# zjykzj/YOLOv4

Measured on AMD Instinct MI355X. Metric: images/sec fwd+bwd @608x608 bs=64 per GPU (YOLOv4 training step: forward + YOLOLoss + backward), higher is better.
Workload: dtype f32

## Files before the change

### yolov4_amd/csrc/conv_planes.hip

```cpp
#include <stdlib.h>
#include <type_traits>
#include "common.h"
#include "conv_geom.h"

namespace {

typedef _Float16 f16x8 __attribute__((ext_vector_type(8)));
typedef float f32x4v __attribute__((ext_vector_type(4)));

__device__ __host__ __forceinline__ unsigned pl_scale_exp(unsigned amax_bits) {
    const unsigned e = (amax_bits >> 23) & 0xffu;
    if (e == 0u || e == 255u) return 127u;
    int se = 268 - (int)e;
    if (se < 2) se = 2;
    if (se > 252) se = 252;
    return (unsigned)se;
}
__device__ __forceinline__ float pl_scale(const unsigned* amax) { return __uint_as_float(pl_scale_exp(amax ? *amax : 0u) << 23); }
__device__ __forceinline__ float pl_unscale(const unsigned* amax) { return __uint_as_float((254u - pl_scale_exp(amax ? *amax : 0u)) << 23); }

struct PlaneConvGeom {
    const unsigned char* src;
    const unsigned char* wt;
    float* dst; long long ldd;
// ... 226 lines not shown
            step(std::integral_constant<int, 0>{}, kt);
            step(std::integral_constant<int, 1>{}, kt + 1);
        }
        if (kt < KT) step(std::integral_constant<int, 0>{}, kt);
    }

    const float un = BF ? 1.0f : pl_unscale(g.src_amax) * pl_unscale(g.wt_amax);
    const float un1 = un * (1.0f / 2048.0f);
    auto result = [&](int i, int j, int e) -> float {
        if constexpr (BF) return acc0[i][j][e];
        else return acc0[i][j][e] * un + acc1[i][j][e] * un1;
    };
    {
        const unsigned drow = (unsigned)g.ldd * 4u, rrow = (unsigned)g.ldr * 4u;
        const long long row0 = (long long)mt * BM;
        const unsigned long long left = (unsigned long long)(g.M - row0);
        const unsigned long long dby = left * drow, rby = g.ldr ? left * rrow : (unsigned long long)g.N * 4ull;
        const __amdgpu_buffer_rsrc_t drs = y4_make_rsrc(reinterpret_cast<char*>(g.dst) + row0 * (long long)drow, (unsigned)(dby < 0xfffffff0ull ? dby : 0xfffffff0ull));
        const __amdgpu_buffer_rsrc_t rrs = y4_make_rsrc(g.res ? reinterpret_cast<const char*>(g.res) + row0 * (long long)rrow : nullptr,
                                                        g.res ? (unsigned)(rby < 0xfffffff0ull ? rby : 0xfffffff0ull) : 0u);
        int lane_e = lane;
        asm volatile("" : "+v"(lane_e));
        const int fr = lane_e & 15, kq = lane_e >> 4;
        const int colb = n0 + wn * WTN + fr;
        const bool allc = n0 + BN <= g.N;
        if constexpr (DG2) {
            const __amdgpu_buffer_rsrc_t xrs = y4_make_rsrc(g.dst, (unsigned)((unsigned long long)g.B * g.Hfull * g.Wfull * drow));
#pragma unroll
            for (int i = 0; i < TM; ++i) {
                const int m0 = mt * BM + wm * WTM + 16 * i + 4 * kq;
                int b = m0 / pix_per_img;
                const int rem = m0 - b * pix_per_img;
                int hc = rem / g.Wd, wc = rem - hc * g.Wd;
#pragma unroll
                for (int e = 0; e < 4; ++e) {
                    const bool rok = m0 + e < g.M;
                    const unsigned po = (unsigned)((b * g.Hfull + 2 * hc + g.cls_ph) * g.Wfull + 2 * wc + g.cls_pw) * drow + (unsigned)colb * 4u;
#pragma unroll
                    for (int j = 0; j < TN; ++j) {
                        const float v = result(i, j, e);
                        const bool cok = rok && (allc || colb + 16 * j < g.N);
                        __builtin_amdgcn_raw_buffer_store_b32(__builtin_bit_cast(unsigned, v), xrs, (int)(cok ? po + 64u * j : 0xffffffffu), 0, PL_ST_POL);
                    }
                    if (++wc == g.Wd) { wc = 0; if (++hc == g.Hd) { hc = 0; ++b; } }
                }
            }
        } else if constexpr (!YB) {
        if (g.res) {
            constexpr int EB = TM > 4 ? 1 : 4;
#pragma unroll
            for (int i = 0; i < TM; ++i) {
                const unsigned rl = (unsigned)(wm * WTM + 16 * i + 4 * kq);
                const unsigned dvo = rl * drow + (unsigned)colb * 4u, rvo = rl * rrow + (unsigned)colb * 4u;
#pragma unroll
                for (int e0 = 0; e0 < 4; e0 += EB) {
                    float rv[EB][TN];
#pragma unroll
                    for (int e = 0; e < EB; ++e)
#pragma unroll
                        for (int j = 0; j < TN; ++j) {
                            const bool cok = allc || colb + 16 * j < g.N;
                            rv[e][j] = __builtin_bit_cast(float, __builtin_amdgcn_raw_buffer_load_b32(rrs, (int)(cok ? rvo + 64u * j : 0xffffffffu), (int)((e0 + e) * rrow), 0));
                        }
#pragma unroll
                    for (int e = 0; e < EB; ++e)
#pragma unroll
                        for (int j = 0; j < TN; ++j) {
                            const float v = result(i, j, e0 + e);
                            acc0[i][j][e0 + e] = v;
                            const bool cok = allc || colb + 16 * j < g.N;
                            __builtin_amdgcn_raw_buffer_store_b32(__builtin_bit_cast(unsigned, v + rv[e][j]), drs, (int)(cok ? dvo + 64u * j : 0xffffffffu), (int)((e0 + e) * drow), PL_ST_POL);
                        }
                }
            }
        } else {
#pragma unroll
            for (int i = 0; i < TM; ++i) {
                const unsigned rl = (unsigned)(wm * WTM + 16 * i + 4 * kq);
                const unsigned dvo = rl * drow + (unsigned)colb * 4u;
#pragma unroll
                for (int e = 0; e < 4; ++e)
#pragma unroll
                    for (int j = 0; j < TN; ++j) {
                        const float v = result(i, j, e);
                        acc0[i][j][e] = v;
                        const bool cok = allc || colb + 16 * j < g.N;
                        __builtin_amdgcn_raw_buffer_store_b32(__builtin_bit_cast(unsigned, v), drs, (int)(cok ? dvo + 64u * j : 0xffffffffu), (int)(e * drow), PL_ST_POL);
                    }
            }
        }
        } else {
            float csum[TN], cssum[TN];
#pragma unroll
            for (int j = 0; j < TN; ++j) { csum[j] = 0.f; cssum[j] = 0.f; }
#pragma unroll
            for (int i = 0; i < TM; ++i) {
                const unsigned rl = (unsigned)(wm * WTM + 16 * i + 4 * kq);
                const unsigned dvo = rl * drow + (unsigned)colb * 2u;
#pragma unroll
                for (int e = 0; e < 4; ++e)
#pragma unroll
                    for (int j = 0; j < TN; ++j) {
                        const float v = result(i, j, e);
                        unsigned u = __builtin_bit_cast(unsigned, v);
                        u = (u + 0x7fffu + ((u >> 16) & 1u)) & 0xffff0000u;
                        const float vr = __builtin_bit_cast(float, u);
                        csum[j] += vr; cssum[j] += vr * vr;
                        const unsigned nb = (unsigned)__builtin_amdgcn_update_dpp(0, (int)u, 0xB1, 0xf, 0xf, true);
                        const bool cok = (allc || colb + 16 * j < g.N) && !(fr & 1);
                        __builtin_amdgcn_raw_buffer_store_b32((u >> 16) | nb, drs, (int)(cok ? dvo + 32u * j : 0xffffffffu), (int)(e * drow), PL_ST_POL);
                    }
                __builtin_amdgcn_sched_barrier(0);
            }
#pragma unroll
            for (int j = 0; j < TN; ++j) { acc0[0][j][0] = csum[j]; acc0[0][j][1] = cssum[j]; }
        }
    }
    if (g.stats) {
        __syncthreads();
        float* red = reinterpret_cast<float*>(smem);
#pragma unroll
        for (int j = 0; j < TN; ++j) {
            float cs = 0.f, css = 0.f;
            if constexpr (YB) {
                cs = acc0[0][j][0]; css = acc0[0][j][1];
            } else {
#pragma unroll
                for (int i = 0; i < TM; ++i)
#pragma unroll
                    for (int e = 0; e < 4; ++e) { const float v = acc0[i][j][e]; cs += v; css += v * v; }
            }
            cs += __shfl_xor(cs, 16, 64); css += __shfl_xor(css, 16, 64);
            cs += __shfl_xor(cs, 32, 64); css += __shfl_xor(css, 32, 64);
            if (kq == 0) {
                const int c = wn * WTN + j * 16 + fr;
                red[(wm * BN + c) * 2 + 0] = cs;
                red[(wm * BN + c) * 2 + 1] = css;
            }
        }
        __syncthreads();
        for (int c = tid; c < BN; c += NTHR) {
            float cs = 0.f, css = 0.f;
#pragma unroll
            for (int w = 0; w < WM; ++w) { cs += red[(w * BN + c) * 2]; css += red[(w * BN + c) * 2 + 1]; }
            const int n = n0 + c;
            if (n < g.N) {
                g.stats[((long long)mt * 2 + 0) * g.N + n] = cs;
                g.stats[((long long)mt * 2 + 1) * g.N + n] = css;
            }
        }
    }
}

struct PlaneWgradGeom {
    const unsigned char* x;
    const unsigned char* dy;
    float* out;
    int B, H, W, Cin, Cout, k, pad, M, J;
    int ldy_ch;
    int ntn, ntj, splits, steps_per_split;
    unsigned long long x_total_bytes, dy_total_bytes;
    const unsigned* x_amax; const unsigned* dy_amax;
};

typedef __fp16 trh4 __attribute__((__vector_size__(4 * sizeof(__fp16))));
__device__ __forceinline__ f16x8 tr_frag(const unsigned char* p) {
    typedef __attribute__((address_space(3))) trh4* lp;
    const trh4 a = __builtin_amdgcn_ds_read_tr16_b64_v4f16((lp)(p));
    const trh4 b = __builtin_amdgcn_ds_read_tr16_b64_v4f16((lp)(p + 4 * PROW));
    f16x8 r;
#pragma unroll
    for (int e = 0; e < 4; ++e) { r[e] = (_Float16)a[e]; r[4 + e] = (_Float16)b[e]; }
    return r;
}

template <int N> __device__ __forceinline__ void pl_wait_vm() {
    static_assert(N == 0 || N == 3 || N == 4 || N == 6 || N == 8 || N == 12, "add the literal");
    if constexpr (N == 0) asm volatile("s_waitcnt vmcnt(0)" ::: "memory");
    else if constexpr (N == 3) asm volatile("s_waitcnt vmcnt(3)" ::: "memory");
    else if constexpr (N == 4) asm volatile("s_waitcnt vmcnt(4)" ::: "memory");
    else if constexpr (N == 6) asm volatile("s_waitcnt vmcnt(6)" ::: "memory");
    else if constexpr (N == 8) asm volatile("s_waitcnt vmcnt(8)" ::: "memory");
    else asm volatile("s_waitcnt vmcnt(12)" ::: "memory");
}

template <int TN_, int TJ_, bool BF, int SD = 1>
__global__ __launch_bounds__(512, 1) void wgrad_planes_mfma(const PlaneWgradGeom g) {
    constexpr int NWAVE = 8, WN2 = 2, WJ = 4;
    constexpr int BAR = 2;
    constexpr int CH = BF ? 64 : 32, CSH = BF ? 6 : 5;
    constexpr int WTN = TN_ / WN2, WTJ = TJ_ / WJ, TM = WTN / 16, TN = WTJ / 16;
    static_assert(TN == 4 && (TM == 4 || (BF && TM == 8)), "wave tile 64 x 64 (bf16 also 128 x 64)");
    constexpr int A_BYTES = (TN_ / CH) * 32 * PROW, B_BYTES = (TJ_ / CH) * 32 * PROW, STAGE = A_BYTES + B_BYTES, NSTAGE = 3;
    constexpr int PA = A_BYTES / 1024 / NWAVE, PB = B_BYTES / 1024 / NWAVE, NDMA = PA + PB;
    static_assert(PA >= 1 && PB >= 1 && (NDMA == 6 || NDMA == 3 || NDMA == 4), "DMA pieces per wave and K-step (counted vmcnt literals)");
    typedef float accv __attribute__((ext_vector_type(4)));
    extern __shared__ __attribute__((aligned(1024))) unsigned char smem[];

    const int tid = threadIdx.x, lane = tid & 63;
    const int wave = __builtin_amdgcn_readfirstlane(tid >> 6);
    const int wn2 = wave >> 2, wj = wave & 3;
    const int tiles = g.ntn * g.ntj;
    int bid = y4_xcd_remap(blockIdx.x, tiles * g.splits);
    const int split = bid / tiles;
    bid -= split * tiles;
    const int tn = bid / g.ntj, tj = bid - tn * g.ntj;
    const int n0 = tn * TN_, j0 = tj * TJ_;
    const int CC = g.Cin >> CSH;

    const int steps_total = (g.M + 31) >> 5;
    const int s0 = split * g.steps_per_split;
    int KT = steps_total - s0;
    if (KT > g.steps_per_split) KT = g.steps_per_split;
    if (KT < 0) KT = 0;
    const long long P0 = (long long)s0 * 32;

    const unsigned pitch_x = (unsigned)g.Cin * 4u, pitch_dy = (unsigned)g.ldy_ch * 4u;
    const long long back = SD == 1 ? (long long)g.pad * g.W + g.pad : 2ll * g.W + 2ll * g.W + 1;
    const long long Pw = SD * SD * P0 > back ? SD * SD * P0 - back : 0;
    const unsigned long long dy_skip = (unsigned long long)P0 * pitch_dy, x_skip = (unsigned long long)Pw * pitch_x;
    const unsigned long long dy_left = g.dy_total_bytes > dy_skip ? g.dy_total_bytes - dy_skip : 0ull;
    const unsigned long long x_left = g.x_total_bytes > x_skip ? g.x_total_bytes - x_skip : 0ull;
    const __amdgpu_buffer_rsrc_t dy_rsrc = y4_make_rsrc(g.dy + dy_skip, (unsigned)(dy_left < 0xfffffff0ull ? dy_left : 0xfffffff0ull));
    const __amdgpu_buffer_rsrc_t x_rsrc = y4_make_rsrc(g.x + x_skip, (unsigned)(x_left < 0xfffffff0ull ? x_left : 0xfffffff0ull));
    const unsigned OOB = 0xffffffffu;

    const int lr = lane >> 3, pos = lane & 7;
    unsigned a_voff[PA];
#pragma unroll
    for (int i = 0; i < PA; ++i) {
        const int a = wave * PA + i;
        const int chunk = a >> 2, p = (a & 3) * 8 + lr;
        const int gsw = ((p >> 1) & 1) | (((p >> 3) & 1) << 1);
        const unsigned srcoff = (unsigned)((((pos >> 1) ^ gsw) << 5) + ((pos & 1) << 4));
        a_voff[i] = (n0 + chunk * CH) < g.Cout ? (unsigned)p * pitch_dy + (unsigned)(n0 / CH + chunk) * 128u + srcoff : OOB;
    }
    const int xp = (wave & 3) * 8 + lr;
    unsigned x_const[PB];
    unsigned x_pk = 0u;
    {
        const int gsw = ((xp >> 1) & 1) | (((xp >> 3) & 1) << 1);
        const unsigned srcoff = (unsigned)((((pos >> 1) ^ gsw) << 5) + ((pos & 1) << 4));
#pragma unroll
        for (int i = 0; i < PB; ++i) {
            const int jg = j0 / CH + (wave >> 2) * PB + i;
            const bool ok = jg * CH < g.J;
            const int tap = ok ? jg / CC : 0;
            const int c32 = jg - tap * CC;
            const int r = tap / g.k, q = tap - r * g.k;
            x_pk |= (unsigned)((ok ? r - g.pad + 2 : 15) | ((q - g.pad + 2) << 4)) << (8 * i);
            x_const[i] = (unsigned)((long long)(SD * SD * P0 - Pw) * pitch_x) + (unsigned)(((r - g.pad) * (SD * g.W) + (q - g.pad)) * (int)pitch_x) +
                         (unsigned)c32 * 128u + srcoff;
        }
    }
    int lp = (int)P0 + xp;
    int lh, lw;
    {
        const long long hw = (long long)g.H * g.W;
        const long long rem = (long long)lp % hw;
        lh = (int)(rem / g.W); lw = (int)(rem - (long long)lh * g.W);
    }
    unsigned lbase = (unsigned)xp * pitch_x;
    unsigned ldy = 0u;
    typedef __attribute__((address_space(3))) void* lds_ptr;
    auto issue = [&](int stage, auto P0c, auto P1c) {
        constexpr int p0 = decltype(P0c)::value, p1 = decltype(P1c)::value;
        unsigned char* st = smem + stage * STAGE;
#pragma unroll
        for (int p = p0; p < p1; ++p) {
            if (p < PA) {
                const unsigned vo = a_voff[p] == OOB ? OOB : a_voff[p] + ldy;
                __builtin_amdgcn_raw_ptr_buffer_load_lds(dy_rsrc, (lds_ptr)(st + (wave * PA + p) * 1024), 16, (int)vo, 0, 0, 0);
            } else {
                const int i = p - PA;
                const int dh = (int)((x_pk >> (8 * i)) & 15u) - 2, dw = (int)((x_pk >> (8 * i + 4)) & 15u) - 2;
                const bool ok = lp < g.M && (unsigned)(SD * lh + dh) < (unsigned)(SD * g.H) && (unsigned)(SD * lw + dw) < (unsigned)(SD * g.W);
                const unsigned lb = SD == 1 ? lbase : (unsigned)(4 * (lp - (int)P0) - 2 * lw) * pitch_x;
                const unsigned vo = ok ? lb + x_const[i] : OOB;
                const int b = ((wave >> 2) * PB + i) * 4 + (wave & 3);
                __builtin_amdgcn_raw_ptr_buffer_load_lds(x_rsrc, (lds_ptr)(st + A_BYTES + b * 1024), 16, (int)vo, 0, 0, 0);
            }
        }
        if constexpr (p1 == NDMA) {
            lp += 32; lbase += 32u * pitch_x; ldy += 32u * pitch_dy;
            lw += 32;
            while (lw >= g.W) { lw -= g.W; if (++lh == g.H) lh = 0; }
        }
    };
    using I0 = std::integral_constant<int, 0>;
    using I6 = std::integral_constant<int, NDMA>;

    accv acc0[TM][TN], acc1[BF ? 1 : TM][BF ? 1 : TN];
#pragma unroll
    for (int i = 0; i < TM; ++i)
#pragma unroll
        for (int j = 0; j < TN; ++j)
#pragma unroll
            for (int e = 0; e < 4; ++e) {
                acc0[i][j][e] = 0.f;
                if constexpr (!BF) acc1[i][j][e] = 0.f;
            }

    const int grp = lane >> 4, qrow = (lane >> 2) & 3, pp = lane & 3;
    const int gsw = ((qrow >> 1) & 1) | ((grp & 1) << 1);
    const int rowoff = (8 * grp + qrow) * PROW + pp * 8;
    int segoff[4];
// ... 222 lines not shown
        const unsigned lrow = (unsigned)(wave * 32 + 4 * fh);
#pragma unroll
        for (int j = 0; j < NT; ++j) {
            const int n = j * 32 + fr;
            const bool nok = n < g.N;
            if constexpr (YB) {
                const bool st = nok && !(fr & 1);
#pragma unroll
                for (int q = 0; q < 4; ++q) {
                    const unsigned vo = st ? (lrow + 8u * q) * drow + (unsigned)n * 2u : 0xffffffffu;
#pragma unroll
                    for (int r = 0; r < 4; ++r) {
                        const unsigned me = (unsigned)pl_bf16_bits(acc[j][q * 4 + r]);
                        const float vr = __uint_as_float(me << 16);
                        cs[j] += vr; css[j] += vr * vr;
                        const unsigned nb = pair_swap_u(me);
                        __builtin_amdgcn_raw_buffer_store_b32(me | (nb << 16), drs, (int)vo, (int)(r * drow), PL_ST_POL);
                    }
                }
            } else {
#pragma unroll
                for (int q = 0; q < 4; ++q) {
                    const unsigned vo = nok ? (lrow + 8u * q) * drow + (unsigned)n * 4u : 0xffffffffu;
                    const unsigned ro = nok ? (lrow + 8u * q) * rrow + (unsigned)n * 4u : 0xffffffffu;
                    float rr[4] = {0.f, 0.f, 0.f, 0.f};
                    if (g.res) {
#pragma unroll
                        for (int r = 0; r < 4; ++r)
                            rr[r] = __builtin_bit_cast(float, __builtin_amdgcn_raw_buffer_load_b32(rrs, (int)ro, (int)(r * rrow), 0));
                    }
#pragma unroll
                    for (int r = 0; r < 4; ++r) {
                        const float v = acc[j][q * 4 + r];
                        cs[j] += v; css[j] += v * v;
                        __builtin_amdgcn_raw_buffer_store_b32(__builtin_bit_cast(unsigned, v + rr[r]), drs, (int)vo, (int)(r * drow), PL_ST_POL);
                    }
                }
            }
        }
    };
    int tile = blockIdx.x;
    if (tile < mtiles) load(ra0, tile);
    while (tile < mtiles) {
        const int t1 = tile + gridDim.x;
        if (t1 < mtiles) load(ra1, t1);
        mma(ra0); epilogue(tile);
        if (t1 >= mtiles) break;
        const int t2 = t1 + gridDim.x;
        if (t2 < mtiles) load(ra0, t2);
        mma(ra1); epilogue(t1);
        tile = t2;
    }
    if (g.stats) {
        __syncthreads();
        float* red = reinterpret_cast<float*>(smem_sb);
#pragma unroll
        for (int j = 0; j < NT; ++j) {
            float a = cs[j], b = css[j];
            a += __shfl_xor(a, 32, 64);
            b += __shfl_xor(b, 32, 64);
            if (fh == 0) { red[(wave * N32 + j * 32 + fr) * 2] = a; red[(wave * N32 + j * 32 + fr) * 2 + 1] = b; }
        }
        __syncthreads();
        for (int c = tid; c < N32; c += NTHR) {
            float a = 0.f, b = 0.f;
#pragma unroll
            for (int w = 0; w < NW; ++w) { a += red[(w * N32 + c) * 2]; b += red[(w * N32 + c) * 2 + 1]; }
            if (c < g.N) {
                g.stats[((long long)blockIdx.x * 2 + 0) * g.N + c] = a;
                g.stats[((long long)blockIdx.x * 2 + 1) * g.N + c] = b;
            }
        }
    }
}

template <int KS, int NT, int NW, bool YB>
static int launch_stream_bf16(const PlaneConvGeom& g0, hipStream_t st, int* nparts) {
    PlaneConvGeom g = g0;
    g.mtiles = (g.M + NW * 32 - 1) / (NW * 32);
    g.ntiles = 1;
    size_t smem = (size_t)NT * 32 * (KS * 32 + 16);
    const size_t red = (size_t)NW * NT * 32 * 2 * sizeof(float);
    if (smem < red) smem = red;
    auto kern = conv1x1_stream_bf16<KS, NT, NW, YB>;
    static Y4DynLds lds_attr;
    if (!lds_attr.ensure(reinterpret_cast<const void*>(kern), smem)) return Y4_ERR_LAUNCH;
    const int resident = NW == 8 ? 256 : 512;
    const int grid = g.mtiles < resident ? g.mtiles : resident;
    if (nparts) *nparts = grid;
    y4::note_kernel("conv1x1_stream_bf16<%d, %d, %d, %s>", KS, NT, NW, YB ? "true" : "false");
    hipLaunchKernelGGL(kern, dim3(grid), dim3(NW * 64), smem, st, g);
    Y4_CHECK_LAUNCH();
    return Y4_OK;
}
static bool stream_bf16_ok(const PlaneConvGeom& g, bool dst_bf16) {
    static const bool off = getenv("Y4_BF_STREAM") && atoi(getenv("Y4_BF_STREAM")) == 0;
    if (off || g.k != 1 || g.stride != 1 || (g.Cs != 64 && g.Cs != 128) || g.N > 128 || g.N < 1) return false;
    if (dst_bf16 && (g.res || (g.N & 1))) return false;
    return g.M >= 128 * 1024;
}
template <bool YB>
static int dispatch_stream_bf16(const PlaneConvGeom& g, hipStream_t st, int* nparts) {
    const int nt = (g.N + 31) / 32;
    if (g.Cs == 64) {
        if (nt == 1) return launch_stream_bf16<4, 1, 4, YB>(g, st, nparts);
        if (nt == 2) return launch_stream_bf16<4, 2, 4, YB>(g, st, nparts);
        return launch_stream_bf16<4, 4, 4, YB>(g, st, nparts);
    }
    if (nt == 1) return launch_stream_bf16<8, 1, 4, YB>(g, st, nparts);
    if (nt == 2) return launch_stream_bf16<8, 2, 4, YB>(g, st, nparts);
    return launch_stream_bf16<8, 4, 4, YB>(g, st, nparts);
}

__global__ __launch_bounds__(256) void bf16_filter_kernel(const float* __restrict__ w, unsigned short* __restrict__ fwd,
                                                          unsigned short* __restrict__ tr, int Cout, int Cin, int kk, int mirror) {
    const long long n = (long long)Cout * kk * Cin;
    const long long i0 = blockIdx.x * (long long)blockDim.x + threadIdx.x, step = (long long)gridDim.x * blockDim.x;
    if (fwd)
        for (long long i = i0; i < n; i += step) fwd[i] = pl_bf16_bits(w[i]);
    if (tr)
        for (long long i = i0; i < n; i += step) {
            const int nn = (int)(i % Cout);
            const long long t = i / Cout;
            const int tp = (int)(t % kk);
            const int tap = mirror ? kk - 1 - tp : tp;
            const int c = (int)(t / kk);
            tr[i] = pl_bf16_bits(w[((long long)nn * kk + tap) * Cin + c]);
        }
}
int bf16_filter(const float* w, unsigned short* fwd, unsigned short* tr, int Cout, int Cin, int kk, bool mirror, hipStream_t st) {
    const long long n = (long long)Cout * kk * Cin;
    const int blocks = (int)((n + 255) / 256 > 2048 ? 2048 : (n + 255) / 256);
    hipLaunchKernelGGL(bf16_filter_kernel, dim3(blocks > 0 ? blocks : 1), dim3(256), 0, st, w, fwd, tr, Cout, Cin, kk, mirror ? 1 : 0);
    Y4_CHECK_LAUNCH();
    return Y4_OK;
}

template <int BM, int BN, int WM, int WN, bool BF, bool YB = false, bool DG2 = false>
int launch_conv_planes(const PlaneConvGeom& g0, hipStream_t st) {
    PlaneConvGeom g = g0;
    g.mtiles = (g.M + BM - 1) / BM;
    g.ntiles = (g.N + BN - 1) / BN;
    constexpr int NW = WM * WN;
    constexpr size_t stage = (size_t)(BM + BN) * PROW;
    constexpr size_t smem = ((NW == 8 && 3 * stage <= 160 * 1024) ? 3ull : 2ull) * stage;
    static_assert(NW == 8 || 2 * smem <= 160 * 1024, "two blocks per CU");
    static_assert(smem <= 160 * 1024, "LDS");
    auto kern = conv_planes_mfma<BM, BN, WM, WN, BF, YB, DG2>;
    static Y4DynLds lds_attr;
    if (!lds_attr.ensure(reinterpret_cast<const void*>(kern), smem)) return Y4_ERR_LAUNCH;
    y4::note_kernel("conv_planes_mfma<%d, %d, %d, %d, %s, %s, %s>", BM, BN, WM, WN, BF ? "true" : "false", YB ? "true" : "false",
                    DG2 ? "true" : "false");
    hipLaunchKernelGGL(kern, dim3(g.mtiles * g.ntiles), dim3(NW * 64), smem, st, g);
    Y4_CHECK_LAUNCH();
    return Y4_OK;
}

}

namespace y4 {

bool planes_conv_ok(int Cin, int Cout, int k, int stride) {
    return Cin > 0 && (Cin & 31) == 0 && Cout > 0 && (Cout & 3) == 0 && (k == 1 || k == 3) && (stride == 1 || stride == 2);
}

static bool conv_window_ok(int B, int Hs, int Ws, int Cs, int N, int k, int stride, bool bf) {
    const int pad = (k - 1) / 2;
    const long long Hd = (Hs + 2 * pad - k) / stride + 1, Wd = (Ws + 2 * pad - k) / stride + 1;
    if (Hd <= 0 || Wd <= 0 || (long long)B * Hd * Wd >= (1ll << 31)) return false;
    const unsigned long long img = (unsigned long long)Hs * Ws * (unsigned long long)Cs * 4ull;
    const unsigned long long wb = (unsigned long long)N * k * k * Cs * (bf ? 2ull : 4ull);
    const unsigned long long imgs_per_tile = 256ull / (unsigned long long)(Hd * Wd) + 2;
    return img * imgs_per_tile < 0xfffffff0ull && wb < 0xfffffff0ull;
}
static bool dgrad_s2_window_ok(int B, int H, int W, int Cin, int Cout, long long lddx) {
    if ((H & 1) || (W & 1)) return false;
    return conv_window_ok(B, H / 2, W / 2, Cout, Cin, 3, 1, false) &&
           (unsigned long long)B * H * W * (unsigned long long)lddx * 4ull < 0xfffffff0ull;
}
static bool wgrad_window_ok(int B, int H, int W, int Cin, int Cout, int k, int stride, bool bf) {
    const long long M = (long long)B * H * W;
    if (M >= (1ll << 31) - 65536) return false;
    if ((unsigned long long)Cout * k * k * Cin * 4ull >= 0xfffffff0ull) return false;
    int ntn, ntj, splits, sps;
    planes_wgrad_plan(B, H, W, Cin, Cout, k, &ntn, &ntj, &splits, &sps, planes_wgrad_tn(Cout, bf), bf);
    const int pad = (k - 1) / 2;
    const unsigned long long range_px = (unsigned long long)sps * 32ull + 2ull * (unsigned long long)(pad * W + pad) + 64ull;
    const unsigned long long range_x = stride == 1 ? range_px : 4ull * range_px + 8ull * (unsigned long long)W + 64ull;
    return range_px * (unsigned long long)Cout * 4ull < 0xfffffff0ull && range_x * (unsigned long long)Cin * 4ull < 0xfffffff0ull;
}
bool planes_fit(int B, int H, int W, int Cin, int Cout, int k, int stride, bool bf, bool dgrad_planes) {
    if (B <= 0 || H <= 0 || W <= 0 || !planes_conv_ok(Cin, Cout, k, stride) || (Cout & 31)) return false;
    if (stride == 2 && (k != 3 || (H & 1) || (W & 1))) return false;
    if (!conv_window_ok(B, H, W, Cin, Cout, k, stride, bf)) return false;
    const int Ho = H / stride, Wo = W / stride;
    if (dgrad_planes) {
        if (stride == 1 ? !conv_window_ok(B, H, W, Cout, Cin, k, 1, bf) : !dgrad_s2_window_ok(B, H, W, Cin, Cout, Cin)) return false;
    }
    return wgrad_window_ok(B, Ho, Wo, Cin, Cout, k, stride, bf);
}

int planes_conv(const void* src, const unsigned* src_amax, const void* wt_planes, const unsigned* wt_amax, float* dst, long long ldd,
                const float* res, long long ldr, float* stats, int* nparts, int B, int Hs, int Ws, int Cs, int N, int k, int stride,
                hipStream_t st, bool bf, bool dst_bf16) {
    PlaneConvGeom g{};
    if (dst_bf16 && (res || (N & 31))) return Y4_ERR_SHAPE;
    g.dst_bf16 = dst_bf16 ? 1 : 0;
    const int pad = (k - 1) / 2;
    g.src = static_cast<const unsigned char*>(src); g.wt = static_cast<const unsigned char*>(wt_planes);
    g.dst = dst; g.ldd = ldd; g.res = res; g.ldr = ldr; g.stats = stats;
    g.B = B; g.Hs = Hs; g.Ws = Ws; g.Cs = Cs; g.N = N; g.k = k; g.stride = stride; g.pad = pad;
    g.Hd = (Hs + 2 * pad - k) / stride + 1;
    g.Wd = (Ws + 2 * pad - k) / stride + 1;
    if (!conv_window_ok(B, Hs, Ws, Cs, N, k, stride, bf)) return Y4_ERR_SHAPE;
    const long long M = (long long)B * g.Hd * g.Wd;
    if (bf && (Cs & 63)) return Y4_ERR_SHAPE;
    g.M = (int)M; g.K = k * k * Cs;
    const unsigned long long img = (unsigned long long)Hs * Ws * (unsigned long long)Cs * 4ull;
    const unsigned long long wb = (unsigned long long)N * g.K * (bf ? 2ull : 4ull);
    g.src_total_bytes = (unsigned long long)B * img;
    g.wt_bytes = (unsigned)wb;
    g.src_amax = src_amax; g.wt_amax = wt_amax;
    static const int small_mode = getenv("Y4_PLANES_SMALL") ? atoi(getenv("Y4_PLANES_SMALL")) : 1;
    bool quant = false;
    {
        const long long nt = (N + 127) / 128;
        const long long b256 = (long long)((g.M + 255) / 256) * nt, b128 = (long long)((g.M + 127) / 128) * nt;
        const long long c256 = ((b256 + 255) / 256) * 2;
        const long long tail = b128 % 512;
        const long long c128 = (b128 / 512) * 2 + (tail == 0 ? 0 : (tail <= 256 ? 1 : 2));
        quant = (double)c128 * 1.08 < (double)c256;
    }
    const bool small = small_mode == 2 || (small_mode == 1 && (g.K <= 256 || quant)) || (small_mode == 4 && g.K <= 256);
    if (bf && stream_bf16_ok(g, dst_bf16)) {
        g.K = Cs;
        return dst_bf16 ? dispatch_stream_bf16<true>(g, st, nparts) : dispatch_stream_bf16<false>(g, st, nparts);
    }
    if (bf) {
        const char* bt = getenv("Y4_BF_TILE");
        const int bf_tile = bt ? atoi(bt) : 0;
        const long long mt = (g.M + 255) / 256;
        const long long r256 = (mt * ((N + 255) / 256) + 255) / 256, r128 = (mt * ((N + 127) / 128) + 255) / 256;
        const bool big = bf_tile == 2 || (bf_tile == 0 && N > 128 && (double)r256 * 2.0 <= (double)r128 * 1.25);
        if (small && !big) {
            if (nparts) *nparts = (g.M + 127) / 128;
            return dst_bf16 ? launch_conv_planes<128, 128, 2, 2, true, true>(g, st) : launch_conv_planes<128, 128, 2, 2, true>(g, st);
        }
        if (nparts) *nparts = (g.M + 255) / 256;
        if (dst_bf16) return big ? launch_conv_planes<256, 256, 2, 4, true, true>(g, st) : launch_conv_planes<256, 128, 4, 2, true, true>(g, st);
        return big ? launch_conv_planes<256, 256, 2, 4, true>(g, st) : launch_conv_planes<256, 128, 4, 2, true>(g, st);
    }
    if (dst_bf16) return Y4_ERR_SHAPE;
    if (nparts) *nparts = small ? (g.M + 127) / 128 : (g.M + 255) / 256;
    return small ? launch_conv_planes<128, 128, 2, 2, false>(g, st) : launch_conv_planes<256, 128, 4, 2, false>(g, st);
}

int planes_dgrad_s2(const void* dy, const unsigned* dy_amax, const void* wt_planes, const unsigned* wt_amax, float* dx, long long lddx,
                    int B, int H, int W, int Cin, int Cout, hipStream_t st, bool bf) {
    if ((H & 1) || (W & 1) || (Cout & 31) || (Cin & 3) || (bf && (Cout & 63))) return Y4_ERR_SHAPE;
    const int Ho = H / 2, Wo = W / 2;
    PlaneConvGeom g{};
    g.src = static_cast<const unsigned char*>(dy); g.wt = static_cast<const unsigned char*>(wt_planes);
    g.dst = dx; g.ldd = lddx;
    g.B = B; g.Hs = Ho; g.Ws = Wo; g.Cs = Cout; g.N = Cin; g.k = 3; g.stride = 1; g.pad = 0;
    g.Hd = Ho; g.Wd = Wo; g.Hfull = H; g.Wfull = W;
    if (B <= 0 || Ho <= 0 || Wo <= 0 || !dgrad_s2_window_ok(B, H, W, Cin, Cout, lddx)) return Y4_ERR_SHAPE;
    const long long M = (long long)B * Ho * Wo;
    g.M = (int)M; g.K = 9 * Cout;
    const unsigned long long img = (unsigned long long)Ho * Wo * (unsigned long long)Cout * 4ull;
    const unsigned long long wb = (unsigned long long)Cin * g.K * (bf ? 2ull : 4ull);
    g.src_total_bytes = (unsigned long long)B * img;
    g.wt_bytes = (unsigned)wb;
    g.src_amax = dy_amax; g.wt_amax = wt_amax;
    for (int c = 3; c >= 0; --c) {
        const int ph = c >> 1, pw = c & 1;
        g.cls_ph = ph; g.cls_pw = pw; g.cls_ntaps = 0;
        for (int r = 0; r < 3; ++r)
            for (int q = 0; q < 3; ++q) {
                if (((ph + 1 - r) & 1) || ((pw + 1 - q) & 1)) continue;
                const int t = g.cls_ntaps++;
                g.cls_dh[t] = (ph + 1 - r) / 2; g.cls_dw[t] = (pw + 1 - q) / 2; g.cls_slot[t] = r * 3 + q;
            }
        const int rc = bf ? launch_conv_planes<256, 128, 4, 2, true, false, true>(g, st)
                          : launch_conv_planes<256, 128, 4, 2, false, false, true>(g, st);
        if (rc != Y4_OK) return rc;
    }
    return Y4_OK;
}

void planes_wgrad_plan(int B, int H, int W, int Cin, int Cout, int k, int* ntn, int* ntj, int* splits, int* sps, int tn, bool bf) {
    static const bool two = !(getenv("Y4_BF_WGRAD_2CU") && atoi(getenv("Y4_BF_WGRAD_2CU")) == 0);
    const int cap = (bf && tn == 128 && two) ? 512 : 256;
    const long long M = (long long)B * H * W;
    const int J = k * k * Cin;
    *ntn = (Cout + tn - 1) / tn;
    *ntj = (J + 255) / 256;
    const int tiles = *ntn * *ntj;
    const long long steps = (M + 31) / 32;
    long long best = -1; int bs = 1;
    for (int s = 1; s <= cap; ++s) {
        const long long per = (steps + s - 1) / s;
        if (s > 1 && per < 12) break;
        const long long rounds = ((long long)tiles * s + cap - 1) / cap;
        const long long cost = rounds * (per + 6);
        if (best < 0 || cost < best) { best = cost; bs = s; }
    }
    const long long per = (steps + bs - 1) / bs;
    *sps = (int)per;
    *splits = (int)((steps + per - 1) / per);
}

int planes_wgrad_tn(int Cout, bool bf) {
    if (!bf) return 128;
    const char* bt = getenv("Y4_BF_WGRAD_TILE");
    const int bf_tile = bt ? atoi(bt) : 0;
    if (bf_tile == 128 || (bf_tile == 256 && Cout >= 256)) return bf_tile;
    return 128;
}

template <int TN_, bool BF, int S = 1>
static int launch_wgrad_planes(const PlaneWgradGeom& g, hipStream_t st) {
    constexpr int CH = BF ? 64 : 32;
    constexpr size_t smem = 3ull * (TN_ / CH + 256 / CH) * 32 * PROW;
    static_assert(smem <= 160 * 1024, "LDS");
    auto kern = wgrad_planes_mfma<TN_, 256, BF, S>;
    static Y4DynLds lds_attr;
    if (!lds_attr.ensure(reinterpret_cast<const void*>(kern), smem)) return Y4_ERR_LAUNCH;
    y4::note_kernel(BF ? "wgrad_planes_mfma<%d, 256, true, %d>" : "wgrad_planes_mfma<%d, 256, false, %d>", TN_, S);
    hipLaunchKernelGGL(kern, dim3(g.ntn * g.ntj * g.splits), dim3(512), smem, st, g);
    Y4_CHECK_LAUNCH();
    return Y4_OK;
}

int planes_wgrad(const void* x, const unsigned* x_amax, const void* dy, const unsigned* dy_amax, float* dw, void* workspace,
                 size_t workspace_bytes, int B, int H, int W, int Cin, int Cout, int k, hipStream_t st, bool bf, int stride) {
    PlaneWgradGeom g{};
    g.x = static_cast<const unsigned char*>(x); g.dy = static_cast<const unsigned char*>(dy);
    if (stride == 2) {
        if (k != 3 || (H & 1) || (W & 1)) return Y4_ERR_SHAPE;
        H /= 2; W /= 2;
    } else if (stride != 1) return Y4_ERR_SHAPE;
    g.B = B; g.H = H; g.W = W; g.Cin = Cin; g.Cout = Cout; g.k = k; g.pad = (k - 1) / 2;
    const long long M = (long long)B * H * W;
    const int q = bf ? 64 : 32;
    g.ldy_ch = (Cout + q - 1) / q * q;
    if (bf && (Cin & 63)) return Y4_ERR_SHAPE;
    if (!wgrad_window_ok(B, H, W, Cin, g.ldy_ch, k, stride, bf)) return Y4_ERR_SHAPE;
    g.M = (int)M; g.J = k * k * Cin;
    const int tn = planes_wgrad_tn(Cout, bf);
    planes_wgrad_plan(B, H, W, Cin, Cout, k, &g.ntn, &g.ntj, &g.splits, &g.steps_per_split, tn, bf);
    g.x_total_bytes = (unsigned long long)M * stride * stride * Cin * 4ull;
    g.dy_total_bytes = (unsigned long long)M * g.ldy_ch * 4ull;
    g.x_amax = x_amax; g.dy_amax = dy_amax;
    const size_t slab = (size_t)Cout * g.J * sizeof(float);
    if (g.splits > 1) {
        if (!workspace || workspace_bytes < slab * g.splits) return Y4_ERR_WORKSPACE;
        g.out = static_cast<float*>(workspace);
    } else {
        g.out = dw;
    }
    int rc;
    if (!bf) rc = stride == 2 ? launch_wgrad_planes<128, false, 2>(g, st) : launch_wgrad_planes<128, false>(g, st);
    else if (stride == 2) rc = tn == 256 ? launch_wgrad_planes<256, true, 2>(g, st) : launch_wgrad_planes<128, true, 2>(g, st);
    else if (tn == 256) rc = launch_wgrad_planes<256, true>(g, st);
    else rc = launch_wgrad_planes<128, true>(g, st);
    if (rc != Y4_OK) return rc;
    if (g.splits > 1) return y4::slab_reduce(static_cast<const float*>(workspace), dw, (long long)Cout * g.J, g.splits, st);
    return Y4_OK;
}

int planes_split(const float* x, long long ld, long long M, int C, const unsigned* amax, void* planes, hipStream_t st, bool bf,
                 long long pitch_ch, int c_valid) {
    const long long pitch = (pitch_ch > 0 ? pitch_ch : (long long)C) * 4;
    const long long total = M * (C / 4);
    const int blocks = (int)((total + 255) / 256 > 4096 ? 4096 : (total + 255) / 256);
    if (bf) {
        hipLaunchKernelGGL(planes_split_bf16_kernel, dim3(blocks > 0 ? blocks : 1), dim3(256), 0, st, x, ld, M, C,
                           static_cast<unsigned char*>(planes), pitch, c_valid > 0 ? c_valid : C);
        Y4_CHECK_LAUNCH();
        return Y4_OK;
    }
    hipLaunchKernelGGL(planes_split_kernel, dim3(blocks > 0 ? blocks : 1), dim3(256), 0, st, x, ld, M, C, amax,
                       static_cast<unsigned char*>(planes), pitch, c_valid > 0 ? c_valid : C);
    Y4_CHECK_LAUNCH();
    return Y4_OK;
}

}

static int g_planes_bf16 = 0;
static inline bool pl_mode_ok() { const int m = y4_get_conv_mode(); return m == 3 || m == 2; }
static inline bool pl_bf() { const int m = y4_get_conv_mode(); return m == 2 || (m == 3 && g_planes_bf16); }

extern "C" {

int y4_set_planes_bf16(int on) { g_planes_bf16 = on ? 1 : 0; return Y4_OK; }
int y4_conv_planes_fit(int B, int H, int W, int Cin, int Cout, int k, int stride, int dgrad_planes) {
    if (!pl_mode_ok()) return 0;
    const bool bf = pl_bf();
    if (bf && ((Cin & 63) || (Cout & 63))) return 0;
    return y4::planes_fit(B, H, W, Cin, Cout, k, stride, bf, dgrad_planes != 0) ? 1 : 0;
}
int y4_get_planes_bf16(void) { return g_planes_bf16; }

int y4_planes_split_f32(const float* x, int ldx, long long M, int C, const unsigned* amax, void* planes, void* stream) {
// ... 129 lines not shown
```

Measured before the change: 456.3.

## Add halo-patch 3x3 stride-1 plane conv kernel reusing input tile across taps

Adds a new MFMA conv kernel for 3x3 stride-1 convolutions on the non-bf16 path. It loads one halo-padded input patch per channel chunk into LDS and reuses it across all nine taps, rather than gathering the input separately for each tap. Filter pieces stream through a two- or three-stage buffer with counted vmcnt waits. It is on by default (env Y4_PLANES_HALO) for non-small shapes whose patch fits in LDS, which cuts global input traffic but adds tight hand-tuned synchronization.

```diff
diff --git a/yolov4_amd/csrc/conv_planes.hip b/yolov4_amd/csrc/conv_planes.hip
--- a/yolov4_amd/csrc/conv_planes.hip
+++ b/yolov4_amd/csrc/conv_planes.hip
@@ -402,6 +402,280 @@
     }
 }
 
+template <int WTM, int TM, int TN, class Result>
+__device__ __forceinline__ void pl_store_f32(const PlaneConvGeom& g, const __amdgpu_buffer_rsrc_t drs, const __amdgpu_buffer_rsrc_t rrs,
+                                             const unsigned drow, const unsigned rrow, const int wm, const int kq, const int colb,
+                                             const bool allc, f32x4v (&acc0)[TM][TN], const Result& result) {
+    if (g.res) {
+        constexpr int EB = TM > 4 ? 1 : 4;
+#pragma unroll
+        for (int i = 0; i < TM; ++i) {
+            const unsigned rl = (unsigned)(wm * WTM + 16 * i + 4 * kq);
+            const unsigned dvo = rl * drow + (unsigned)colb * 4u, rvo = rl * rrow + (unsigned)colb * 4u;
+#pragma unroll
+            for (int e0 = 0; e0 < 4; e0 += EB) {
+                float rv[EB][TN];
+#pragma unroll
+                for (int e = 0; e < EB; ++e)
+#pragma unroll
+                    for (int j = 0; j < TN; ++j) {
+                        const bool cok = allc || colb + 16 * j < g.N;
+                        rv[e][j] = __builtin_bit_cast(float, __builtin_amdgcn_raw_buffer_load_b32(rrs, (int)(cok ? rvo + 64u * j : 0xffffffffu), (int)((e0 + e) * rrow), 0));
+                    }
+#pragma unroll
+                for (int e = 0; e < EB; ++e)
+#pragma unroll
+                    for (int j = 0; j < TN; ++j) {
+                        const float v = result(i, j, e0 + e);
+                        acc0[i][j][e0 + e] = v;
+                        const bool cok = allc || colb + 16 * j < g.N;
+                        __builtin_amdgcn_raw_buffer_store_b32(__builtin_bit_cast(unsigned, v + rv[e][j]), drs, (int)(cok ? dvo + 64u * j : 0xffffffffu), (int)((e0 + e) * drow), PL_ST_POL);
+                    }
+            }
+        }
+    } else {
+#pragma unroll
+        for (int i = 0; i < TM; ++i) {
+            const unsigned rl = (unsigned)(wm * WTM + 16 * i + 4 * kq);
+            const unsigned dvo = rl * drow + (unsigned)colb * 4u;
+#pragma unroll
+            for (int e = 0; e < 4; ++e)
+#pragma unroll
+                for (int j = 0; j < TN; ++j) {
+                    const float v = result(i, j, e);
+                    acc0[i][j][e] = v;
+                    const bool cok = allc || colb + 16 * j < g.N;
+                    __builtin_amdgcn_raw_buffer_store_b32(__builtin_bit_cast(unsigned, v), drs, (int)(cok ? dvo + 64u * j : 0xffffffffu), (int)(e * drow), PL_ST_POL);
+                }
+        }
+    }
+}
+template <int BN, int WM, int WTN, int NTHR, int TM, int TN>
+__device__ __forceinline__ void pl_column_sums(const PlaneConvGeom& g, unsigned char* smem, const int mt, const int n0, const int wm,
+                                               const int wn, f32x4v (&acc0)[TM][TN]) {
+    const int tid = threadIdx.x, fr = tid & 15, kq = (tid & 63) >> 4;
+    __syncthreads();
+    float* red = reinterpret_cast<float*>(smem);
+#pragma unroll
+    for (int j = 0; j < TN; ++j) {
+        float cs = 0.f, css = 0.f;
+#pragma unroll
+        for (int i = 0; i < TM; ++i)
+#pragma unroll
+            for (int e = 0; e < 4; ++e) { const float v = acc0[i][j][e]; cs += v; css += v * v; }
+        cs += __shfl_xor(cs, 16, 64); css += __shfl_xor(css, 16, 64);
+        cs += __shfl_xor(cs, 32, 64); css += __shfl_xor(css, 32, 64);
+        if (kq == 0) {
+            const int c = wn * WTN + j * 16 + fr;
+            red[(wm * BN + c) * 2 + 0] = cs;
+            red[(wm * BN + c) * 2 + 1] = css;
+        }
+    }
+    __syncthreads();
+    for (int c = tid; c < BN; c += NTHR) {
+        float cs = 0.f, css = 0.f;
+#pragma unroll
+        for (int w = 0; w < WM; ++w) { cs += red[(w * BN + c) * 2]; css += red[(w * BN + c) * 2 + 1]; }
+        const int n = n0 + c;
+        if (n < g.N) {
+            g.stats[((long long)mt * 2 + 0) * g.N + n] = cs;
+            g.stats[((long long)mt * 2 + 1) * g.N + n] = css;
+        }
+    }
+}
+template <int N> __device__ __forceinline__ void pl_wait_vm_upto4() {
+    static_assert(N >= 0 && N <= 4, "add the literal");
+    if constexpr (N == 0) asm volatile("s_waitcnt vmcnt(0)" ::: "memory");
+    else if constexpr (N == 1) asm volatile("s_waitcnt vmcnt(1)" ::: "memory");
+    else if constexpr (N == 2) asm volatile("s_waitcnt vmcnt(2)" ::: "memory");
+    else if constexpr (N == 3) asm volatile("s_waitcnt vmcnt(3)" ::: "memory");
+    else asm volatile("s_waitcnt vmcnt(4)" ::: "memory");
+}
+
+template <int BM, int BN, int WM, int WN, int PW, int NSB>
+__global__ __launch_bounds__(WM * WN * 64, 1) void conv_planes_halo_mfma(const PlaneConvGeom g) {
+    constexpr int NWAVE = WM * WN, NTHR = NWAVE * 64;
+    constexpr int WTM = BM / WM, WTN = BN / WN, TM = WTM / 16, TN = WTN / 16;
+    constexpr int P_BYTES = PW * NWAVE * 1024, B_BYTES = BN * PROW, B_AT = 2 * P_BYTES;
+    constexpr int PB = BN / 8 / NWAVE;
+    static_assert(NWAVE == 8 && PB == 2 && PW >= 1 && PW <= 8 && (NSB == 2 || NSB == 3) && TM >= 2,
+                  "the counted vmcnt below assumes 2 filter pieces and at most one patch piece per wave and K-tile");
+    static_assert(NSB == 2 || PW <= 7, "three filter stages: the last patch piece must go out before tap 7's filter pieces");
+    static_assert(B_AT + NSB * B_BYTES <= 160 * 1024, "LDS");
+    extern __shared__ __attribute__((aligned(1024))) unsigned char smem[];
+
+    const int tid = threadIdx.x, lane = tid & 63;
+    const int wave = __builtin_amdgcn_readfirstlane(tid >> 6);
+    const int wm = wave / WN, wn = wave % WN;
+    const int lt = y4_xcd_remap(blockIdx.x, g.mtiles * g.ntiles);
+    const int mt = lt / g.ntiles, nt = lt - mt * g.ntiles;
+    const int n0 = nt * BN;
+    const int CC = g.Cs >> 5;
+
+    const unsigned H = (unsigned)g.Hs, W = (unsigned)g.Ws, W1 = W + 1u, S1 = (H + 1u) * W1;
+    const unsigned pix_per_img = H * W;
+    const unsigned m_first = (unsigned)mt * BM;
+    const unsigned b_first = m_first / pix_per_img;
+    const unsigned b_last = (m_first + (BM - 1)) / pix_per_img - b_first;
+    int P0;
+    {
+        const unsigned rem = m_first - b_first * pix_per_img;
+        const unsigned h0 = rem / W;
+        P0 = (int)(h0 * W1 + (rem - h0 * W)) - (int)(W1 + 1u);
+    }
+    const unsigned pitch = (unsigned)g.Cs * 4u;
+    const unsigned long long img_bytes = (unsigned long long)pix_per_img * pitch;
+    const unsigned long long skip = (unsigned long long)b_first * img_bytes;
+    const unsigned long long left = g.src_total_bytes > skip ? g.src_total_bytes - skip : 0ull;
+    const __amdgpu_buffer_rsrc_t src_rsrc = y4_make_rsrc(g.src + skip, (unsigned)(left < 0xfffffff0ull ? left : 0xfffffff0ull));
+    const __amdgpu_buffer_rsrc_t wt_rsrc = y4_make_rsrc(g.wt, g.wt_bytes);
+    const unsigned OOB = 0xffffffffu;
+
+    const int lr = lane >> 3, pos = lane & 7;
+    unsigned p_voff[PW];
+#pragma unroll
+    for (int i = 0; i < PW; ++i) {
+        const int p = (i * NWAVE + wave) * 8 + lr;
+        const int I = P0 + p;
+        const unsigned Iu = I < 0 ? 0u : (unsigned)I;
+        const unsigned b = Iu / S1;
+        const unsigned rem = Iu - b * S1;
+        const unsigned h = rem / W1, w = rem - h * W1;
+        const bool ok = I >= 0 && b <= b_last && b_first + b < (unsigned)g.B && h < H && w < W;
+        const unsigned chunk = (unsigned)(pos ^ ((p >> 1) & 7));
+        unsigned vo = ok ? ((b * H + h) * W + w) * pitch + chunk * 16u : OOB;
+        asm volatile("" : "+v"(vo));
+        p_voff[i] = vo;
+    }
+    unsigned b_off[PB];
+#pragma unroll
+    for (int j = 0; j < PB; ++j) {
+        const int row = (wave * PB + j) * 8 + lr;
+        const int chunk = pos ^ ((row >> 1) & 7);
+        b_off[j] = (n0 + row) < g.N ? (unsigned)(n0 + row) * (unsigned)g.K * 4u + (unsigned)chunk * 16u : OOB;
+    }
+    typedef __attribute__((address_space(3))) void* lds_ptr;
+    auto issue_patch = [&](const int i, const int cc) {
+        __builtin_amdgcn_raw_ptr_buffer_load_lds(src_rsrc, (lds_ptr)(smem + (cc & 1) * P_BYTES + (i * NWAVE + wave) * 1024), 16,
+                                                 (int)p_voff[i], (int)((unsigned)cc * 128u), 0, 0);
+    };
+    auto issue_filter = [&](const int stage, const int tap, const int cc) {
+        const unsigned soff = (unsigned)(tap * CC + cc) * 128u;
+#pragma unroll
+        for (int j = 0; j < PB; ++j)
+            __builtin_amdgcn_raw_ptr_buffer_load_lds(wt_rsrc, (lds_ptr)(smem + B_AT + stage * B_BYTES + (wave * PB + j) * 1024), 16,
+                                                     (int)b_off[j], (int)soff, 0, 0);
+    };
+
+    f32x4v acc0[TM][TN], acc1[TM][TN];
+#pragma unroll
+    for (int i = 0; i < TM; ++i)
+#pragma unroll
+        for (int j = 0; j < TN; ++j)
+#pragma unroll
+            for (int e = 0; e < 4; ++e) { acc0[i][j][e] = 0.f; acc1[i][j][e] = 0.f; }
+
+    const int fr = lane & 15, kq = lane >> 4;
+    int a_row[TM];
+#pragma unroll
+    for (int i = 0; i < TM; ++i) {
+        const unsigned m = m_first + (unsigned)(wm * WTM + i * 16 + fr);
+        const unsigned b = m / pix_per_img;
+        const unsigned rem = m - b * pix_per_img;
+        const unsigned h = rem / W;
+        a_row[i] = (int)((b - b_first) * S1 + h * W1 + (rem - h * W)) - P0;
+    }
+    const int swb = (fr >> 1) & 7;
+    const int b_hi = B_AT + (wn * WTN + fr) * PROW + ((kq ^ swb) << 4), b_lo = B_AT + (wn * WTN + fr) * PROW + (((4 + kq) ^ swb) << 4);
+
+    auto step = [&](auto TC, const int c, const bool more) {
+        constexpr int t = decltype(TC)::value;
+        const int stage = NSB == 3 ? t % 3 : ((c + t) & 1);
+        const unsigned char* fbase = smem + stage * B_BYTES;
+        const int tapoff = (t / 3 - 1) * (int)W1 + (t % 3 - 1);
+        const int pbuf = (c & 1) * P_BYTES;
+        auto a_at = [&](const int i) -> int {
+            int row = a_row[i];
+            asm volatile("" : "+v"(row));
+            row += tapoff;
+            return pbuf + row * PROW + ((kq ^ ((row >> 1) & 7)) << 4);
+        };
+        f16x8 fb[TN][2];
+#pragma unroll
+        for (int j = 0; j < TN; ++j) {
+            fb[j][0] = *reinterpret_cast<const f16x8*>(fbase + b_hi + j * 16 * PROW);
+            fb[j][1] = *reinterpret_cast<const f16x8*>(fbase + b_lo + j * 16 * PROW);
+        }
+        f16x8 fap[2][2];
+        {
+            const int a0 = a_at(0);
+            fap[0][0] = *reinterpret_cast<const f16x8*>(smem + a0);
+            fap[0][1] = *reinterpret_cast<const f16x8*>(smem + (a0 ^ 64));
+        }
+#pragma unroll
+        for (int i = 0; i < TM; ++i) {
+            if (i + 1 < TM) {
+                const int an = a_at(i + 1);
+                fap[(i + 1) & 1][0] = *reinterpret_cast<const f16x8*>(smem + an);
+                fap[(i + 1) & 1][1] = *reinterpret_cast<const f16x8*>(smem + (an ^ 64));
+            }
+            const f16x8 fa0 = fap[i & 1][0], fa1 = fap[i & 1][1];
+            if (i == TM - 1) {
+                __builtin_amdgcn_sched_barrier(0);
+                asm volatile("s_waitcnt lgkmcnt(0)" ::: "memory");
+                if (more || t < 8) {
+                    constexpr int pt = t < PW ? 1 : 0, pt1 = (t >= 1 && t - 1 < PW) ? 1 : 0;
+                    if (more) pl_wait_vm_upto4<NSB == 3 ? pt1 + 2 + pt : pt>();
+                    else pl_wait_vm_upto4<(NSB == 3 && t + 2 <= 8) ? 2 : 0>();
+                    __builtin_amdgcn_s_barrier();
+                    if (more || t + NSB <= 8) issue_filter(stage, (t + NSB) % 9, c + (t + NSB) / 9);
+                }
+            }
+#pragma unroll
+            for (int j = 0; j < TN; ++j) {
+                acc1[i][j] = pl_mma<false>(fa1, fb[j][0], acc1[i][j]);
+                acc1[i][j] = pl_mma<false>(fa0, fb[j][1], acc1[i][j]);
+                acc0[i][j] = pl_mma<false>(fa0, fb[j][0], acc0[i][j]);
+            }
+            if constexpr (t < PW) {
+                if (i == 0 && more) issue_patch(t, c + 1);
+            }
+        }
+    };
+
+#pragma unroll
+    for (int i = 0; i < PW; ++i) issue_patch(i, 0);
+    for (int s = 0; s < NSB; ++s) issue_filter(s, s, 0);
+    pl_wait_vm_upto4<PB * (NSB - 1)>();
+    __builtin_amdgcn_s_barrier();
+    for (int c = 0; c < CC; ++c) {
+        const bool more = c + 1 < CC;
+        step(std::integral_constant<int, 0>{}, c, more); step(std::integral_constant<int, 1>{}, c, more);
+        step(std::integral_constant<int, 2>{}, c, more); step(std::integral_constant<int, 3>{}, c, more);
+        step(std::integral_constant<int, 4>{}, c, more); step(std::integral_constant<int, 5>{}, c, more);
+        step(std::integral_constant<int, 6>{}, c, more); step(std::integral_constant<int, 7>{}, c, more);
+        step(std::integral_constant<int, 8>{}, c, more);
+    }
+
+    const float un = pl_unscale(g.src_amax) * pl_unscale(g.wt_amax);
+    const float un1 = un * (1.0f / 2048.0f);
+    auto result = [&](int i, int j, int e) -> float { return acc0[i][j][e] * un + acc1[i][j][e] * un1; };
+    {
+        const unsigned drow = (unsigned)g.ldd * 4u, rrow = (unsigned)g.ldr * 4u;
+        const long long row0 = (long long)mt * BM;
+        const unsigned long long rows_left = (unsigned long long)(g.M - row0);
+        const unsigned long long dby = rows_left * drow, rby = g.ldr ? rows_left * rrow : (unsigned long long)g.N * 4ull;
+        const __amdgpu_buffer_rsrc_t drs = y4_make_rsrc(reinterpret_cast<char*>(g.dst) + row0 * (long long)drow, (unsigned)(dby < 0xfffffff0ull ? dby : 0xfffffff0ull));
+        const __amdgpu_buffer_rsrc_t rrs = y4_make_rsrc(g.res ? reinterpret_cast<const char*>(g.res) + row0 * (long long)rrow : nullptr,
+                                                        g.res ? (unsigned)(rby < 0xfffffff0ull ? rby : 0xfffffff0ull) : 0u);
+        int lane_e = lane;
+        asm volatile("" : "+v"(lane_e));
+        const int colb = n0 + wn * WTN + (lane_e & 15);
+        pl_store_f32<WTM>(g, drs, rrs, drow, rrow, wm, lane_e >> 4, colb, n0 + BN <= g.N, acc0, result);
+    }
+    if (g.stats) pl_column_sums<BN, WM, WTN, NTHR>(g, smem, mt, n0, wm, wn, acc0);
+}
+
 struct PlaneWgradGeom {
     const unsigned char* x;
     const unsigned char* dy;
@@ -930,6 +1204,31 @@
     y4::note_kernel("conv_planes_mfma<%d, %d, %d, %d, %s, %s, %s>", BM, BN, WM, WN, BF ? "true" : "false", YB ? "true" : "false",
                     DG2 ? "true" : "false");
     hipLaunchKernelGGL(kern, dim3(g.mtiles * g.ntiles), dim3(NW * 64), smem, st, g);
+    Y4_CHECK_LAUNCH();
+    return Y4_OK;
+}
+
+int halo_patch_rows(int H, int W, int BM) {
+    const long long lw = (BM - 2) / W + 1, iw = (BM - 2) / ((long long)H * W) + 1;
+    const long long rows = BM + lw + iw * (W + 1) + 2ll * (W + 2);
+    return rows > 1 << 20 ? 1 << 20 : (int)rows;
+}
+bool halo_measured_faster(const PlaneConvGeom& g, bool small) {
+    return !small;
+}
+template <int PW, int NSB>
+int launch_conv_planes_halo(const PlaneConvGeom& g0, hipStream_t st) {
+    constexpr int BM = 256, BN = 128;
+    PlaneConvGeom g = g0;
+    g.mtiles = (g.M + BM - 1) / BM;
+    g.ntiles = (g.N + BN - 1) / BN;
+    constexpr size_t smem = 2ull * PW * 8 * 1024 + (size_t)NSB * BN * PROW;
+    static_assert(smem <= 160 * 1024, "LDS");
+    auto kern = conv_planes_halo_mfma<BM, BN, 4, 2, PW, NSB>;
+    static Y4DynLds lds_attr;
+    if (!lds_attr.ensure(reinterpret_cast<const void*>(kern), smem)) return Y4_ERR_LAUNCH;
+    y4::note_kernel("conv_planes_halo_mfma<%d, %d, 4, 2, %d, %d>", BM, BN, PW, NSB);
+    hipLaunchKernelGGL(kern, dim3(g.mtiles * g.ntiles), dim3(512), smem, st, g);
     Y4_CHECK_LAUNCH();
     return Y4_OK;
 }
@@ -1029,6 +1328,16 @@
         return big ? launch_conv_planes<256, 256, 2, 4, true>(g, st) : launch_conv_planes<256, 128, 4, 2, true>(g, st);
     }
     if (dst_bf16) return Y4_ERR_SHAPE;
+    if (k == 3 && stride == 1) {
+        const char* hv = getenv("Y4_PLANES_HALO");
+        const int halo_mode = hv ? atoi(hv) : 1;
+        const int rows = halo_patch_rows(Hs, Ws, 256);
+        const bool fits = rows <= 8 * 64;
+        if (fits && (halo_mode == 2 || (halo_mode == 1 && halo_measured_faster(g, small)))) {
+            if (nparts) *nparts = (g.M + 255) / 256;
+            return rows <= 6 * 64 ? launch_conv_planes_halo<6, 3>(g, st) : launch_conv_planes_halo<8, 2>(g, st);
+        }
+    }
     if (nparts) *nparts = small ? (g.M + 127) / 128 : (g.M + 255) / 256;
     return small ? launch_conv_planes<128, 128, 2, 2, false>(g, st) : launch_conv_planes<256, 128, 4, 2, false>(g, st);
 }
```

Result: no change. 460.3, median of 6 (+0.9%).
